# nelpy/ghost

Hardware: AMD Instinct MI355X
Metric: Msamples/s CWT (128ch x 1e6 samp x 100 scales); % HBM roofline; 1/2/4/8 GPU (higher is better)
Workload: dtype f32

## Files before the change

ghost_amd/csrc/api.cpp:

```cpp
#include <hip/hip_runtime.h>

#include <algorithm>
#include <cmath>
#include <cstdio>
#include <cstdlib>
#include <cstring>
#include <exception>
#include <map>
#include <new>
#include <string>
#include <vector>

#include "../../include/ghostcwt.h"
#include "../../include/ghostcwt_debug.h"
#include <memory>

#include "errors.h"
#include "host_out.h"
#include "interp.h"
#include "kernels.h"
#include "morse_exact.h"
#include "morlet_exact.h"
#include "options.h"
#include "planner.h"
// ... 1038 lines not shown
      }
      if (p->detect) {
        hipEvent_t bands_done;
        int rc_ = get_event(p, &bands_done);
        if (rc_) return rc_;
        he = hipEventRecord(bands_done, st);
        if (he == hipSuccess) he = hipStreamWaitEvent(p->det_stream, bands_done, 0);
        if (he != hipSuccess) return hip_err(he, "detector fork");
        he = launch_band_sums(p->d_hist, P1, p->d_bands, slots, p->det_stream);
        if (he != hipSuccess) return hip_err(he, "launch_band_sums");
        he = launch_precision_predict(p->d_bands, p->d_gain, p->d_scale_level, p->d_scale_length, p->ep_dev[ep.batch_first].pred_levels, S,
                                      (int)hp.levels.size(), (double)Pt, p->kappa_eps, p->oob_tol, p->d_pred, nullptr, nullptr, slots, psegs,
                                      p->det_stream);
        if (he != hipSuccess) return hip_err(he, "launch_precision_predict");
        p->last_batch_slots = slots; p->last_batch = ep.batch_first; p->last_pt = (double)Pt; p->last_rows = P1;
      }
    } else if (A > 1) {
      return set_err(GCWT_ERR_UNSUPPORTED, "internal: long mode without the float64 forward transform");
    } else {
    RUN(ST_FWD, launch_fft_cols_batch(dx, p->d_x, P1, kRowLen, N, P, P1 > 1 ? P : 0, p->d_tw4096,
                                      fast_fft ? p->d_tw256 : nullptr, p->d_sums, inv_n, sin, nb, st,
                                      rows_a));
    RUN(ST_FWD, launch_fft_rows(-1, p->d_x, p->d_x, kRowLen, rows_a, kRowLen, kRowLen, P, P, 0,
                                p->d_tw4096, fast_fft ? p->d_tw256 : nullptr, 1.0f, slots, st,
                                hp.n_fullband > 0 ? kRowLen : kRowLen / 2, hermitian ? P1 : 0));
    }
    const bool fused_blocks = p->fuse_blocks && p->synth_kernel == 7 && !p->use_synth16;
    const bool side = p->level_streams && hp.levels.size() > 2;
    const EpochDev& dev = p->ep_dev[ep.batch_first];
    std::vector<char> in_h(hp.levels.size(), 0);
    bool any_h = false;
    for (size_t l = 0; l < hp.levels.size(); ++l)
      if (level_kernel(p, hp.levels[l]) == LK_INTERP) {
        in_h[hp.levels[l].xr_owner >= 0 ? (size_t)hp.levels[l].xr_owner : l] = 1;
        any_h = true;
      }
    for (size_t l = 0; l < hp.levels.size(); ++l)
      if (hp.levels[l].xr_owner >= 0) in_h[l] = in_h[(size_t)hp.levels[l].xr_owner];
    const bool early = side && p->early_interp && p->profiling != 1 && !p->synth_streams && any_h &&
                       dev.n_items_i + dev.n_items_p[0] + dev.n_items_p[1] > 0;
    std::vector<int> stream_of(hp.levels.size(), 0);
    if (side) {
      double load[3] = {0.0, 0.0, 0.0};
      std::vector<size_t> order;
      for (size_t l = 0; l < hp.levels.size(); ++l)
        if (hp.levels[l].xr_owner == (int)l && !(early && in_h[l])) order.push_back(l);
      std::stable_sort(order.begin(), order.end(), [&](size_t a, size_t b) { return ep.lv[a].m > ep.lv[b].m; });
      const int k0 = early ? 1 : 0;
      for (size_t l : order) {
        const int k = (int)(std::min_element(load + k0, load + 3) - load);
        stream_of[l] = k;
        load[k] += 40e-6 + 32.0 * (double)ep.lv[l].m * (double)slots / 4.5e12;
      }
      for (size_t l = 0; l < hp.levels.size(); ++l) stream_of[l] = stream_of[hp.levels[l].xr_owner];
    }
    bool forked[2] = {false, false};
    hipEvent_t spectrum_ready = nullptr;
    if (side) {
      int rc_ = get_event(p, &spectrum_ready);
      if (rc_) return rc_;
      he = hipEventRecord(spectrum_ready, st);
      if (he != hipSuccess) return hip_err(he, "hipEventRecord");
    }
    for (size_t li = 0; li < (early ? 2 : 1) * hp.levels.size(); ++li) {
      const size_t l = li % hp.levels.size();
      if (early && (in_h[l] != 0) != (li < hp.levels.size())) continue;
      const LevelPlan& lp = hp.levels[l];
      const EpochLevel& el = ep.lv[l];
      float2* xr = p->d_xr + el.xr_offset;
      hipStream_t ls = st;
      RowTaper taper;
      if (p->high_precision && lp.taper_hi > 0.0 && lp.band_shift == 0) {
        const double k1 = lp.taper_hi * (double)Pt / (2.0 * M_PI), k0 = 0.5 * k1;
        if (k1 - k0 >= 1.0) { taper.p1 = P1; taper.k0 = (float)k0; taper.inv_width = (float)(1.0 / (k1 - k0)); }
      }
      if (side) {
        const int k = stream_of[l];
        ls = k == 0 ? st : p->aux[k - 1];
        if (k > 0 && !forked[k - 1]) {
          he = hipStreamWaitEvent(ls, spectrum_ready, 0);
          if (he != hipSuccess) return hip_err(he, "hipStreamWaitEvent");
          forked[k - 1] = true;
        }
        p->cur = ls;
      }
      if (lp.xr_owner != (int)l) {
      } else if (lp.decimation / A <= kMaxTwoPassDecimation) {
        const int Q = kRowLen * A / lp.decimation;
        const float2* src = p->d_x;
        int64_t src_row = kRowLen, src_cstride = P;
        if (lp.band_shift > 0) {
          const int64_t U = (int64_t)lp.band_shift * el.m / hp.block;
          if (U % P1 != 0 || U / P1 > Q) return set_err(GCWT_ERR_INVALID, "internal: band shift does not slice the spectrum");
          float2* xs = p->d_xs + (int64_t)stream_of[l] * slots * p->xs_stride;
          RUN(ST_DECIM, launch_shift_gather(p->d_x, xs, P1, Q, (int)(U / P1), kRowLen, P, p->xs_stride, slots, ls));
          src = xs; src_row = Q; src_cstride = p->xs_stride;
        }
        RUN(ST_DECIM, launch_fft_rows(+1, src, xr, Q, P1, src_row, Q, src_cstride, hp.max_xr,
                                      P1 > 1 ? el.m : 0, p->d_tw4096,
                                      fast_fft ? p->d_tw256 : nullptr, 1.0f, slots, ls, 0, 0, taper));
        if (P1 > 1)
          RUN(ST_DECIM, launch_fft_cols(+1, false, xr, xr, P1, Q, hp.max_xr, hp.max_xr, 0,
                                        p->d_tw4096, fast_fft ? p->d_tw256 : nullptr, p->d_sums,
                                        inv_n, 0, slots, ls));
      } else {
        const int n1 = (int)std::min<int64_t>(P1, el.m);
        const int q = (int)(el.m / n1);
        RUN(ST_DECIM, launch_level_small(p->d_x, xr, n1, q, kRowLen, P, hp.max_xr, p->d_tw4096, slots, ls, taper));
      }
      const float scale = (float)(1.0 / ((double)hp.block * (double)Pt));
      const LevelKernel lk = level_kernel(p, lp);
      if (lk == LK_SYNTH16 || (lk == LK_SYNTH7 && !fused_blocks))
        RUN(ST_BLOCK, launch_block_fft(xr, p->d_xb + el.xb_offset, el.m, lp.hop, lp.halo, el.blk_lo,
                                       el.nblk, hp.max_xr, hp.max_xb, p->d_tw256, scale, slots, ls));
    }
    if (side) p->cur = nullptr;
    auto join_levels = [&]() -> int {
      for (int k = 0; k < 2; ++k) {
        if (!forked[k]) continue;
        forked[k] = false;
        hipEvent_t done;
        int rc_ = get_event(p, &done);
        if (rc_) return rc_;
        he = hipEventRecord(done, p->aux[k]);
        if (he == hipSuccess) he = hipStreamWaitEvent(st, done, 0);
        if (he != hipSuccess) return hip_err(he, "level streams join");
      }
      return GCWT_OK;
    };
    if (!early) {
      int rc_ = join_levels();
      if (rc_) return rc_;
    }
    hipStream_t si = st;
    if (dev.n_items_i > 0) {
      const bool beside = p->synth_streams && (dev.n_items7 > 0 || dev.n_items7w > 0 || dev.n_items7n > 0 || dev.n_items > 0);
      if (beside) {
        hipEvent_t levels_done;
        int rc_ = get_event(p, &levels_done);
        if (rc_) return rc_;
        he = hipEventRecord(levels_done, st);
        if (he == hipSuccess) he = hipStreamWaitEvent(p->aux[0], levels_done, 0);
        if (he != hipSuccess) return hip_err(he, "synthesis fork");
        si = p->aux[0];
      }
      SynthiArgs ai{};
      ai.tw256 = p->d_tw256;
      ai.level_tw = p->d_level_tw;
      ai.items = dev.items_i;
      ai.levels = dev.levels_i;
      ai.scale_list = p->d_scale_list;
      ai.scale_aux = p->d_scale_aux;
      ai.gain = p->d_gain;
      ai.coef = p->d_interp_coef;
      ai.out = dout;
      ai.row_len = row_len;
      ai.xr = p->d_xr;
      ai.xr_cstride = hp.max_xr;
      ai.xb_scale = (float)(1.0 / ((double)hp.block * (double)Pt));
      ai.n_scales = S;
      ai.channels_fastest = p->interp_grid >= 0 ? p->interp_grid : (slots <= 32 ? 1 : 0);
      if (dev.n_items_i > 65535) ai.channels_fastest = 0;
      ai.seg = sout;
      p->cur = si;
      for (int part = 0; part < 2; ++part) {
        const int first = part == 0 ? 0 : dev.split_i, n_part = part == 0 ? dev.split_i : dev.n_items_i - dev.split_i;
        if (n_part == 0) continue;
        ai.items = dev.items_i + first;
        if (strided) RUN(ST_INTERP, launch_synthis(mode, ai, n_part, slots, si));
        else RUN(ST_INTERP, launch_synthi(mode, ai, n_part, slots, si));
      }
      p->cur = nullptr;
    }
    for (int k = 0; k < 2; ++k) {
      if (dev.n_items_p[k] == 0) continue;
      SynthpArgs ap{};
      ap.tw256 = p->d_tw256;
      ap.level_tw = p->d_level_tw;
      ap.items = dev.items_p[k];
      ap.levels = dev.levels_p;
      ap.scale_list = p->d_scale_list;
      ap.scale_aux = p->d_scale_aux;
      ap.gain_lv = p->d_gain_lv;
      ap.level_half_tw = p->d_half_tw;
      ap.coef = p->d_interp_coef;
      ap.out = dout;
      ap.row_len = row_len;
      ap.xr = p->d_xr;
      ap.xr_cstride = hp.max_xr;
      ap.xb_scale = (float)(1.0 / ((double)hp.block * (double)Pt));
      ap.n_scales = S;
      ap.channels_fastest = p->interp_grid >= 0 ? p->interp_grid : (slots <= 32 ? 1 : 0);
      if (dev.n_items_p[k] > 65535) ap.channels_fastest = 0;
      ap.flags = 0;
      ap.seg = sout;
      p->cur = si;
#ifdef GCWT_MEASURE
      if (strided) return set_err(GCWT_ERR_UNSUPPORTED, "output stride with the pipelined interpolating kernel");
      RUN(ST_INTERP, launch_synthp(mode, ap, dev.n_items_p[k], slots, k == 1, si));
#else
      return set_err(GCWT_ERR_INVALID, "internal: a level planned for the measure build's pipelined kernel");
#endif
      p->cur = nullptr;
    }
    if (early) {
      int rc_ = join_levels();
      if (rc_) return rc_;
    }
    if (dev.n_items > 0) {
      SynthArgs a{};
      a.xb = p->d_xb;
      a.bank = p->d_bank;
      a.tw256 = p->d_tw256;
      a.level_tw = p->d_level_tw;
      a.items = dev.items;
      a.levels = dev.levels;
      a.out = dout;
      a.xb_cstride = hp.max_xb;
      a.row_len = row_len;
      a.n_scales = S;
      a.seg = sout;
      RUN(ST_SYNTH, launch_synth(mode, a, dev.n_items, slots, st));
    }
    for (int variant = 0; variant < 3; ++variant) {
      const int wide = variant == 2;
      const int cols7 = variant == 0 ? 16 : p->synth_cols;
      const int n7 = variant == 0 ? dev.n_items7n : wide ? dev.n_items7w : dev.n_items7;
      if (n7 == 0) continue;
      Synth7Args a7{};
      a7.xb = p->d_xb;
      a7.bank = p->d_bank;
      a7.tw256 = p->d_tw256;
      a7.level_tw = p->d_level_tw;
      a7.items = variant == 0 ? dev.items7n : wide ? dev.items7w : dev.items7;
      a7.levels = dev.levels7;
      a7.scale_list = p->d_scale_list;
      a7.gain = p->d_gain;
      a7.gain_lv = p->d_gain_lv;
      a7.level_half_tw = p->d_half_tw;
      a7.complex_gains = hp.morlet ? 1 : 0;
      a7.out = dout;
      a7.xb_cstride = hp.max_xb;
      a7.row_len = row_len;
      a7.n_scales = S;
      a7.drop_stores = p->drop_stores;
      a7.seg = sout;
      a7.clock_probe = p->d_probe;
      if (fused_blocks) {
        a7.xr = p->d_xr;
        a7.xr_cstride = hp.max_xr;
        a7.xb_scale = (float)(1.0 / ((double)hp.block * (double)Pt));
      }
      if (strided) {
        RUN(ST_SYNTH, launch_synth7s(mode, cols7, a7, n7, slots, st));
        continue;
      }
#ifdef GCWT_MEASURE
      if (p->synth_kernel == 8 && variant == 1)
        RUN(ST_SYNTH, launch_synth8(mode, p->synth_cols, a7, n7, slots, st));
      else
#endif
        RUN(ST_SYNTH, launch_synth7(mode, cols7, wide != 0, a7, n7, slots, st));
    }
    if (si != st) {
      hipEvent_t interp_done;
      int rc_ = get_event(p, &interp_done);
      if (rc_) return rc_;
      he = hipEventRecord(interp_done, si);
      if (he == hipSuccess) he = hipStreamWaitEvent(st, interp_done, 0);
      if (he != hipSuccess) return hip_err(he, "synthesis join");
    }
    if (p->detect && p->d_y) {
      hipEvent_t pred_done;
      int rc_ = get_event(p, &pred_done);
      if (rc_) return rc_;
      he = hipEventRecord(pred_done, p->det_stream);
      if (he == hipSuccess) he = hipStreamWaitEvent(st, pred_done, 0);
      if (he != hipSuccess) return hip_err(he, "detector join");
    }
    if (p->profiling && !hp.levels.empty()) p->last.synth_launches++;
    auto response = [&](int i, int scratch, const float2** h_out) -> int {
      const auto cached = p->hfull_cache.find({i, P1});
      if (cached != p->hfull_cache.end()) { *h_out = cached->second; return GCWT_OK; }
      float2* dst = p->d_hfull + (int64_t)scratch * hp.max_p;
      float2* keep = nullptr;
      const int64_t bytes = (int64_t)sizeof(float2) * P;
      if (!p->hfull_cache_full && p->hfull_cache_bytes + bytes <= p->fullband_cache_cap) {
        if (hipMalloc((void**)&keep, (size_t)bytes) == hipSuccess) dst = keep;
        else {
          (void)hipGetLastError();
          p->hfull_cache_full = true;
        }
      }
      {
        SpanGuard sg_(p, ST_FULLBAND);
        int rc_ = sg_.rc;
        if (!rc_) {
          he = launch_fullband_filter(dst, p->d_bank_sc, i, p->d_amps, P1, st);
          if (he != hipSuccess) rc_ = hip_err(he, "launch_fullband_filter");
        }
        if (!rc_) rc_ = sg_.end();
        if (rc_) { if (keep) (void)hipFree(keep); return rc_; }
      }
      if (keep) {
        p->hfull_cache[{i, P1}] = keep;
        p->hfull_cache_bytes += bytes;
// ... 697 lines not shown
```

ghost_amd/csrc/kernels.h:

```cpp
#pragma once
#include <hip/hip_runtime.h>

#include <algorithm>
#include <cstdint>

#include "../../include/ghostcwt.h"

namespace gcwt {

constexpr int kRowLenDev = 4096;

#ifdef GCWT_MEASURE
constexpr bool kMeasureBuild = true;
#else
constexpr bool kMeasureBuild = false;
#endif

struct BankScale {
  double omega;
  double half_delay;
  int64_t length;
  int64_t amp_offset;
  int32_t bin_lo, n_bins;
  int32_t decimation;
// ... 17 lines not shown

inline int direct_front_pad(int64_t length) { return (int)((7 - (length - 1) / 2) & 7); }

constexpr int kSegBatch = 16;
struct SegIn {
  int64_t x_off[kSegBatch];
  int64_t n_valid[kSegBatch];
  int64_t n_lead[kSegBatch];
  int64_t ramp_lo[kSegBatch], ramp_hi[kSegBatch];
  int32_t n_channels, pad;
};
struct OutStride {
  int64_t r0 = 0;
  int64_t c0 = 0;
  int32_t k = 1;
  uint32_t magic = 0;
};
inline OutStride make_out_stride(int64_t k, int64_t r0) {
  OutStride o;
  o.r0 = r0;
  o.k = (int32_t)k;
  o.c0 = (r0 + k - 1) / k;
  o.magic = k > 1 ? (uint32_t)((((uint64_t)1 << 32) + (uint64_t)k - 1) / (uint64_t)k) : 0u;
  return o;
}
__device__ __forceinline__ bool stride_keep(const OutStride& o, int64_t n, int64_t* col) {
  const uint32_t t = (uint32_t)n;
  const uint32_t q = __umulhi(t, o.magic);
  *col = (int64_t)q - o.c0;
  return n >= 0 && q * (uint32_t)o.k == t;
}

struct SegOut {
  int64_t seg_col[kSegBatch];
  int64_t w_lo[kSegBatch];
  int64_t w_hi[kSegBatch];
  int32_t n_channels, pad;
  OutStride os;
};

struct SynthItemDev {
  int32_t level, scale, blk0, nblk;
};

struct SynthLevelDev {
  int32_t decimation, hop, halo, blk_base;
  int64_t xb_offset;
  int64_t tw_offset;
};

struct SynthArgs {
  const float2* xb;
  const float2* bank;
  const float2* tw256;
  const float2* level_tw;
  const SynthItemDev* items;
  const SynthLevelDev* levels;
  float* out;
  int64_t xb_cstride;
  int64_t row_len;
  int32_t n_scales;
  int32_t pad;
  SegOut seg;
};

struct Synth7Item {
  int32_t level, blk0, rtile, pad;
};

struct Synth7Level {
  int32_t decimation, log2r, hop, halo, nblk, n_scales, scale_offset, blk_base;
  int32_t n_plain;
  int32_t half_offset;
  int32_t band_shift;
  int32_t pad1;
  int64_t xb_offset;
  int64_t tw_offset;
  int64_t xr_offset;
  int64_t m_mask;
};

struct Synth7Args {
  const float2* xb;
  const float2* bank;
  const float2* tw256;
  const float2* level_tw;
  const Synth7Item* items;
  const Synth7Level* levels;
  const int32_t* scale_list;
  const float* gain;
  const float* gain_lv;
  const float2* level_half_tw;
  float* out;
  int64_t xb_cstride;
  int64_t row_len;
  const float2* xr;
  int64_t xr_cstride;
  float xb_scale;
  int32_t complex_gains;
  unsigned long long* clock_probe;
  int32_t n_scales;
  int32_t drop_stores;
  SegOut seg;
};

__host__ __device__ constexpr int synth7_ex_elem(int lg, int colw, int j) {
  return ((colw >> lg) << (4 + lg)) + (colw & ((1 << lg) - 1)) + (j << lg);
}
__host__ __device__ constexpr bool synth7_exchange_wave_local(int ncol, int R) { return R <= ncol && 16 * R <= 64; }
constexpr bool synth7_exchange_spans_one_wave(int ncol, int lg) {
  for (int colw = 0; colw < ncol; ++colw)
    for (int j = 0; j < 16; ++j)
      if ((16 * colw) >> 6 != synth7_ex_elem(lg, colw, j) >> 6) return false;
  return true;
}
constexpr int kSynth7LocalStride = 4;
#define GCWT_EX_CHECK(ncol, lg, local)                                                                    \
  static_assert(synth7_exchange_wave_local(ncol, 1 << (lg)) == (local) &&                                 \
                    ((1 << (lg)) > (ncol) || synth7_exchange_spans_one_wave(ncol, lg) == (local)) &&      \
                    (((1 << (lg)) > (ncol) ? (ncol) : (1 << (lg))) <= kSynth7LocalStride) == (local),     \
                "k_synth7: the wave-local predicate does not match the column mapping")
GCWT_EX_CHECK(16, 0, true);  GCWT_EX_CHECK(16, 1, true);  GCWT_EX_CHECK(16, 2, true);  GCWT_EX_CHECK(16, 3, false);
GCWT_EX_CHECK(16, 4, false); GCWT_EX_CHECK(16, 5, false); GCWT_EX_CHECK(16, 6, false);
GCWT_EX_CHECK(32, 0, true);  GCWT_EX_CHECK(32, 1, true);  GCWT_EX_CHECK(32, 2, true);  GCWT_EX_CHECK(32, 3, false);
GCWT_EX_CHECK(32, 4, false); GCWT_EX_CHECK(32, 5, false); GCWT_EX_CHECK(32, 6, false); GCWT_EX_CHECK(32, 7, false);
#undef GCWT_EX_CHECK

hipError_t launch_synth7(int mode, int ncol, bool wide_halo, const Synth7Args& a, int n_items, int n_channels,
                         hipStream_t st);
hipError_t launch_synth7s(int mode, int ncol, const Synth7Args& a, int n_items, int n_channels, hipStream_t st);

struct SynthiItem {
  int32_t level, blk0;
  int32_t pass0, n_pass;
  int32_t wt_lo, wt_hi;
};
struct SynthiLevel {
  int32_t decimation, q, log2q, factor;
  int32_t hop, halo, nblk, n_scales, scale_offset, blk_base;
  int32_t log2nb, taps;
  int64_t tw_offset;
  int64_t xr_offset;
  int64_t m_mask;
  int64_t coef_offset;
};
struct SynthiArgs {
  const float2* tw256;
  const float2* level_tw;
  const SynthiItem* items;
  const SynthiLevel* levels;
  const int32_t* scale_list;
  const int32_t* scale_aux;
  const float* gain;
  const float* coef;
  float* out;
  int64_t row_len;
  const float2* xr;
  int64_t xr_cstride;
  float xb_scale;
  int32_t n_scales;
  int32_t channels_fastest;
  SegOut seg;
};
hipError_t launch_synthi(int mode, const SynthiArgs& a, int n_items, int n_channels, hipStream_t st);
hipError_t launch_synthis(int mode, const SynthiArgs& a, int n_items, int n_channels, hipStream_t st);
constexpr int kSynthpThreads = 512;
constexpr int kSynthpProducers = 2;
constexpr int kSynthpSlots = 4;
constexpr int kSynthpMaxFactor = 256;
struct SynthpItem {
  int32_t level, blk0;
  int32_t round0, n_rounds;
};
struct SynthpLevel {
  int32_t decimation, factor;
  int32_t hop, halo, nblk, n_scales, scale_offset, blk_base;
  int32_t log2nb;
  int32_t n_plain;
  int32_t half_offset;
  int32_t help;
  int64_t tw_offset;
  int64_t xr_offset;
  int64_t m_mask;
  int64_t coef_offset;
};
struct SynthpArgs {
  const float2* tw256;
  const float2* level_tw;
  const SynthpItem* items;
  const SynthpLevel* levels;
  const int32_t* scale_list;
  const int32_t* scale_aux;
  const float* gain_lv;
  const float2* level_half_tw;
  const float* coef;
  float* out;
  int64_t row_len;
  const float2* xr;
  int64_t xr_cstride;
  float xb_scale;
  int32_t n_scales;
  int32_t channels_fastest;
  int32_t flags;
  int32_t pad0;
  SegOut seg;
};
hipError_t launch_synthp(int mode, const SynthpArgs& a, int n_items, int n_channels, bool exact0, hipStream_t st);
hipError_t launch_synth8(int mode, int ncol, const Synth7Args& a, int n_items, int n_channels,
                         hipStream_t st);

hipError_t dft_f64(const double* x, int64_t n, int is_complex, int inverse, double* out);
hipError_t fastconv_f64(const double* signal, int64_t n, int signal_is_complex, const double* kernel, int64_t m,
                        int kernel_is_complex, int64_t first, int64_t count, double* out);

hipError_t rows_to_host(const float* d_src, int64_t src_pitch, int64_t n_rows, int64_t row_elems, void* dst,
                        int64_t dst_pitch, bool widen, bool pinned);

constexpr int kSumParts = 256;
constexpr int kSumPartsOwn = 64;
constexpr size_t channel_sum_doubles(size_t n_channels) { return n_channels * (kSumParts + 1); }
hipError_t launch_channel_sum(const float* x, int64_t n, int n_channels, double* sums,
                              hipStream_t st);
hipError_t launch_build_bank(float2* bank, float* gain, const BankScale* sc, const double* amps,
                             int n_scales, int B, hipStream_t st);
constexpr int kScaleIndexMask = 0x00FFFFFF;
hipError_t launch_scale_windows(const float* gain, int32_t* scale_list, int n_listed, float tol,
                                float* gain_lv, bool prune, hipStream_t st);
hipError_t launch_gain_rows_complex(const float2* bank, const int32_t* scale_list, int n_listed, float2* gain_lv,
                                    hipStream_t st);
hipError_t launch_bank_gain(const float2* bank, float* gain, const BankScale* sc, int n_scales,
                            hipStream_t st);
hipError_t launch_fullband_filter(float2* h, const BankScale* sc, int scale, const double* amps,
                                  int p1, hipStream_t st);
hipError_t launch_fullband_mul(const float2* x, const float2* h, float2* z, int64_t p, int n_slots,
                               hipStream_t st);
constexpr int kFullbandSet = 4;
struct FullbandSet {
  const float2* h[kFullbandSet];
  float2* z[kFullbandSet];
  int32_t n, pad;
};
hipError_t launch_fullband_rows(const float2* x, const FullbandSet& set, int p1, int64_t x_cstride, int64_t z_cstride,
                                const float2* twt, const float2* tw256, int n_slots, hipStream_t st,
                                int group = 0);
bool fullband_cols_fused(int p1);
constexpr int kFullband4Scales = 8;
hipError_t launch_fullband4(int mode, const float2* x, const float2* const* h, const int32_t* scales, int n, float* out,
                            int64_t x_cstride, const float2* twt, const float2* tw256, int n_scales, int64_t row_len,
                            const SegOut& seg, int n_slots, hipStream_t st);
hipError_t launch_fullband_cols(int mode, const float2* z, float* out, int p1, int64_t z_cstride,
                                const float2* tw4096, const float2* tw256, int scale, int n_scales,
                                int64_t row_len, const SegOut& seg, int n_slots, hipStream_t st);
hipError_t launch_fullband_store(int mode, const float2* y, float* out, int64_t p, int scale,
                                 int n_scales, int64_t row_len, const SegOut& seg, int n_segments,
                                 hipStream_t st);
hipError_t launch_build_direct(float2* psi, const DirectScale* sc, int n_direct, int64_t max_len,
                               const double* amps, float2* tail, float2* psi_literal, hipStream_t st);
hipError_t launch_fft_cols(int sign, bool real_in, const void* in, float2* out, int len, int ld,
                           int64_t in_cstride, int64_t out_cstride, int64_t tw_n,
                           const float2* tw4096, const float2* tw256, const double* sums, double inv_n, int64_t n_valid,
                           int n_channels, hipStream_t st, int64_t n_lead = 0, int rows_out = 0);
hipError_t launch_fft_cols_batch(const float* in, float2* out, int len, int ld, int64_t in_cstride,
                                 int64_t out_cstride, int64_t tw_n, const float2* tw4096,
                                 const float2* tw256, const double* sums, double inv_n,
                                 const SegIn& segs, int n_segments, hipStream_t st, int rows_out);
struct RowTaper {
  int32_t p1 = 0;
  float k0 = 0.f, inv_width = 0.f;
};
hipError_t launch_fft_rows(int sign, const float2* in, float2* out, int len, int64_t n_rows,
                           int64_t in_ld, int64_t out_ld, int64_t in_cstride, int64_t out_cstride,
                           int64_t tw_n, const float2* tw4096, const float2* tw256, float scale,
                           int n_channels, hipStream_t st, int out_len = 0, int mirror = 0,
                           RowTaper taper = RowTaper());
void fwd64_fill_tables(double2* host);
hipError_t launch_fwd64_cols(const float* in, double2* y, int p1, int64_t in_cstride, int64_t y_cstride,
                             int64_t p, const double2* tables, const double* sums, double inv_n,
                             const SegIn& segs, int n_segments, int rows_out, hipStream_t st, int in_stride = 1,
                             int in_offset = 0, bool fold_mean = false);
hipError_t launch_channel_sum_final(double* sums, int n_channels, int parts, hipStream_t st);
constexpr int fold_parts(int p1) { return p1 == 256 ? 32 : 256; }
hipError_t launch_fwd64_rows(const double2* y, float2* x, int n_rows, int64_t y_cstride, int64_t x_cstride,
                             const double2* tables, int n_slots, int out_len, int mirror, hipStream_t st,
                             int comb_a = 0, int comb_n = 1, int64_t p_true = 0, float* hist = nullptr, int hist_rows = 0,
                             const double* fold_sums = nullptr, double inv_n = 0.0, int64_t n_valid = 0, int p1 = 0);

constexpr int kSpecBands = 16 * 24;
__host__ __device__ inline int spec_band(float k) {
  union { float f; uint32_t u; } b;
  b.f = k;
  const int v = (int)(b.u >> 19) - 127 * 16;
  return v < 0 ? 0 : (v >= kSpecBands ? kSpecBands - 1 : v);
}
struct PredSegs {
  int32_t seg[kSegBatch];
  int32_t n_channels, pad;
};
struct PredLevel {
  int32_t decimation;
  int32_t band_shift;
  float k0, k1;
};
constexpr int kRowBands = 128;
hipError_t launch_band_sums(const float* hist, int p1, float* bands, int n_slots, hipStream_t st);
hipError_t launch_precision_predict(const float* bands, const float* gain, const int32_t* scale_level,
                                    const int32_t* scale_length, const PredLevel* levels, int n_scales, int n_levels, double p_true,
// ... 50 lines not shown
```

ghost_amd/csrc/synthi.hip:

```cpp
#include <hip/hip_runtime.h>

#include <type_traits>

#include "interp.h"
#include "kernels.h"
#include "options.h"
#include "synth_math.h"

#ifndef GCWT_STORE_AUX
#define GCWT_STORE_AUX 2
#endif

namespace gcwt {

namespace {
constexpr int kT = kInterpTaps;
static_assert(kT == 8, "the FIR loop below is written for 8 taps");
constexpr int kColsI = kInterpCols;
constexpr int kLgColsI = kColsI == 32 ? 5 : kColsI == 16 ? 4 : 3;
constexpr int kThreadsI = 16 * kColsI;
constexpr int kWavesI = kThreadsI / 64;
constexpr int kPlaneI = kThreadsI + 1;
constexpr int kZPad = 4;
constexpr int kSlotsMax = kColsI / 2;
static_assert(kColsI == kInterpCols, "the host cuts the passes for this many columns (interp.h)");
constexpr int kZElems = 256 * kColsI + kSlotsMax * kZPad;
constexpr int kExElems = kZElems > 16 * kPlaneI ? kZElems : 16 * kPlaneI;
constexpr int kGainRowI = 16 * 20;
constexpr int kLdsBytes = kExElems * 8 + 256 * 8 + kSlotsMax * kGainRowI * 4 + 2 * 256 * 4;

__device__ __forceinline__ v2f fir_mul_re(v2f z, v2f c) {
  v2f r;
  asm("v_pk_mul_f32 %0, %1, %2 op_sel:[0,0] op_sel_hi:[0,1]" : "=v"(r) : "v"(z), "v"(c));
  return r;
}
__device__ __forceinline__ v2f fir_mul_im(v2f z, v2f c) {
  v2f r;
  asm("v_pk_mul_f32 %0, %1, %2 op_sel:[1,0] op_sel_hi:[1,1]" : "=v"(r) : "v"(z), "v"(c));
  return r;
}
__device__ __forceinline__ v2f fir_fma_re(v2f acc, v2f z, v2f c) {
  v2f r;
  asm("v_pk_fma_f32 %0, %1, %2, %3 op_sel:[0,0,0] op_sel_hi:[0,1,1]" : "=v"(r) : "v"(z), "v"(c), "v"(acc));
  return r;
}
__device__ __forceinline__ v2f fir_fma_im(v2f acc, v2f z, v2f c) {
  v2f r;
  asm("v_pk_fma_f32 %0, %1, %2, %3 op_sel:[1,0,0] op_sel_hi:[1,1,1]" : "=v"(r) : "v"(z), "v"(c), "v"(acc));
  return r;
}
__device__ __forceinline__ v2f pk_mul(v2f a, v2f b) {
  v2f r;
  asm("v_pk_mul_f32 %0, %1, %2" : "=v"(r) : "v"(a), "v"(b));
  return r;
}
__device__ __forceinline__ v2f pk_fma(v2f a, v2f b, v2f c) {
  v2f r;
  asm("v_pk_fma_f32 %0, %1, %2, %3" : "=v"(r) : "v"(a), "v"(b), "v"(c));
  return r;
}
template <int J0, int J1>
__device__ __forceinline__ void fir_taps(const v2f* zp, const v2f (&cf)[2][kT], v2f (&are)[2], v2f (&aim)[2]) {
  {
    const v2f w = zp[J0];
#pragma unroll
    for (int pr = 0; pr < 2; ++pr) { are[pr] = fir_mul_re(w, cf[pr][J0]); aim[pr] = fir_mul_im(w, cf[pr][J0]); }
  }
#pragma unroll
  for (int j = J0 + 1; j < J1; ++j) {
    const v2f w = zp[j];
#pragma unroll
    for (int pr = 0; pr < 2; ++pr) { are[pr] = fir_fma_re(are[pr], w, cf[pr][j]); aim[pr] = fir_fma_im(aim[pr], w, cf[pr][j]); }
  }
}
}

template <int MODE>
__global__ void __launch_bounds__(kThreadsI, kColsI == 32 ? 4 : 3) k_synthi(const SynthiArgs a) {
  extern __shared__ __attribute__((aligned(16))) char smem[];
  v2f* const ex = reinterpret_cast<v2f*>(smem);
  v2f* const twl = ex + kExElems;
  float* const stage = reinterpret_cast<float*>(twl + 256);
  int* const sc_lds = reinterpret_cast<int*>(stage + kSlotsMax * kGainRowI);
  int* const aux_lds = sc_lds + 256;

  const SynthiItem it = a.items[a.channels_fastest ? blockIdx.y : blockIdx.x];
  const SynthiLevel lv = a.levels[it.level];
  const int c = a.channels_fastest ? blockIdx.x : blockIdx.y;
  const int seg = c / a.seg.n_channels, ch = c - seg * a.seg.n_channels;
  const int R = lv.decimation, q = lv.q, lgq = lv.log2q, hop = lv.hop, halo = lv.halo;
  const int lgnb = lv.log2nb, nb = 1 << lgnb;
  const int64_t n_b = (int64_t)(lv.blk_base + it.blk0) * hop * R;
  const int64_t w_lo = a.seg.w_lo[seg];
  const int64_t w_len = a.seg.w_hi[seg] - w_lo;
  if (n_b + (int64_t)nb * hop * R <= w_lo || n_b >= w_lo + w_len) return;

  const int tid = threadIdx.x, lane = tid & 63;
  const int wave = __builtin_amdgcn_readfirstlane(tid >> 6);
  const int colw = tid >> 4, t = tid & 15;
  const int lgns = kLgColsI - lgq - lgnb, ns = 1 << lgns;
  const int zslot = colw >> lgq, p = colw & (q - 1);
  const int slot = zslot & (ns - 1), blk_l = zslot >> lgns;
  const int nzs = kColsI >> lgq;
  const int n_scales = lv.n_scales;
  const int* const scales = a.scale_list + lv.scale_offset;
  const int* const auxs = a.scale_aux + lv.scale_offset;
  for (int i = tid; i < n_scales; i += kThreadsI) { sc_lds[i] = scales[i]; aux_lds[i] = auxs[i]; }
  if (tid < 256) {
    const float2 w = a.tw256[tid];
    twl[tid] = (v2f){w.x, w.y};
  }
  auto stage_slot = [&](int i) { return (i >> 8) * kGainRowI + (i & 15) * 20 + ((i >> 4) & 15); };
  for (int i = tid; i < ns * 256; i += kThreadsI) {
    const int sb = min(it.pass0 * ns + (i >> 8), n_scales - 1);
    stage[stage_slot(i)] = a.gain[(int64_t)(scales[sb] & kScaleIndexMask) * 256 + (i & 255)];
  }

  v2f* const fx = ex;
  v2f* const xbs = ex + kSlotsMax * 256;
  {
    v2f v[16];
    if (colw < nb) {
      const int64_t base = (int64_t)(lv.blk_base + min(it.blk0 + colw, lv.nblk - 1)) * hop - halo + t;
      const float2* xr = a.xr + (int64_t)c * a.xr_cstride + lv.xr_offset;
#pragma unroll
      for (int j = 0; j < 16; ++j) {
        const float2 u = xr[(base + 16 * j) & lv.m_mask];
        v[j] = (v2f){u.x, -u.y};
      }
      idft16v(v);
#pragma unroll
      for (int m = 0; m < 16; ++m) {
        const float2 w = a.tw256[(t * m) & 255];
        fx[colw * 256 + t * 16 + (m ^ t)] = cmulv(v[dft16_pos(m)], (v2f){w.x, w.y});
      }
    }
    __syncthreads();
    if (colw < nb) {
#pragma unroll
      for (int k1 = 0; k1 < 16; ++k1) v[k1] = fx[colw * 256 + k1 * 16 + (t ^ k1)];
      idft16v(v);
#pragma unroll
      for (int j = 0; j < 16; ++j) {
        const v2f z = v[dft16_pos(j)];
        xbs[colw * 256 + t + 16 * j] = (v2f){z.x * a.xb_scale, -z.y * a.xb_scale};
      }
    }
    __syncthreads();
  }
  v2f pw[16];
  {
    const int r = p * lv.factor;
    const float2* ltw = a.level_tw + lv.tw_offset;
    const float2 b0 = ltw[t * r], st = ltw[16 * r];
    v2f wcur = (v2f){b0.x, b0.y};
    const v2f wstep = (v2f){st.x, st.y};
#pragma unroll
    for (int j = 0; j < 16; ++j) {
      pw[j] = cmulv(xbs[blk_l * 256 + t + 16 * j], wcur);
      wcur = cmulv(wcur, wstep);
    }
  }

  const int a2 = tid >> kLgColsI, col2 = tid & (kColsI - 1);
  const int zslot2 = col2 >> lgq, p2 = col2 & (q - 1);
  const int zstride = (256 << lgq) + kZPad;
  v2f* const zw = ex + zslot2 * zstride + (a2 << lgq) + p2;

  const int I = lv.factor;
  const bool six = lv.taps == 6;
  int lgi4 = 0;
  while ((4 << lgi4) < I) ++lgi4;
  const int tps = hop * (R >> 2);
  const int n_wt = it.wt_hi - it.wt_lo;
  static_assert(GCWT_SYNTHI_COLS != 16 || (kWavesI == 4 && kInterpMaxFactor <= 1024),
                "a wave's lane-tasks keep their class mod I / 4 (the 8- and 32-column measurement builds: I <= 256 only)");
  const float* const coef_lv = a.coef + lv.coef_offset;
  constexpr int kElem = 1;
  const unsigned ext_bytes = w_len > 0 ? (unsigned)(w_len * (4 * kElem)) : 0u;
  float* const out0 = a.out + ((int64_t)ch * a.n_scales * a.row_len + a.seg.seg_col[seg] + w_lo) * kElem;
  const int s_base = (int)(n_b - w_lo);
  const int pass_end = it.pass0 + it.n_pass;
  int cur_par = -1;
  v2f cf[2][kT];
  __syncthreads();

  for (int pass = it.pass0; pass < pass_end; ++pass) {
    const int b0 = pass * ns;
    const bool has_next = pass + 1 < pass_end;
    float nxt[kSlotsMax];
    if (has_next) {
#pragma unroll
      for (int u = 0; u < kSlotsMax; ++u) {
        const int i = tid + kThreadsI * u;
        if (i < ns * 256) {
          const int sb = min(b0 + ns + (i >> 8), n_scales - 1);
          nxt[u] = a.gain[(int64_t)(sc_lds[sb] & kScaleIndexMask) * 256 + (i & 255)];
        }
      }
    }
    {
      const int bs = min(b0 + slot, n_scales - 1);
      const int entry = sc_lds[bs];
      const int kc = aux_lds[bs] & 0xffff;
      const float4* const hs = reinterpret_cast<const float4*>(stage + slot * kGainRowI + t * 20);
      v2f v[16];
      unsigned cut = (unsigned)__builtin_amdgcn_readfirstlane(entry) >> 24;
      if (q == 2) {
        const int other = sc_lds[min(b0 + (((colw ^ 2) >> lgq) & (ns - 1)), n_scales - 1)];
        cut = min(cut, (unsigned)__builtin_amdgcn_readfirstlane(min((unsigned)entry >> 24, (unsigned)other >> 24)));
        cut = (unsigned)__builtin_amdgcn_readfirstlane(cut);
      }
      switch (cut) {
#define GCWT_WINDOW(hi) case 16 - (hi): gain_first_layer<hi>(v, pw, hs); break;
        GCWT_WINDOW(15) GCWT_WINDOW(14) GCWT_WINDOW(13) GCWT_WINDOW(12) GCWT_WINDOW(11) GCWT_WINDOW(10) GCWT_WINDOW(9)
#undef GCWT_WINDOW
        default: gain_first_layer<16>(v, pw, hs); break;
      }
      idft16v_tail(v);
      const unsigned step8 = (unsigned)((t - kc) & 255) << 3;
      unsigned idx8 = (unsigned)((-(kc >> lgq) * p) & 255) << 3;
      v2f* const exw = ex + ((t - kc) & 15) * kPlaneI + colw;
      const char* const twb = reinterpret_cast<const char*>(twl);
#pragma unroll
      for (int j = 0; j < 16; ++j) {
        exw[j * kColsI] = cmulv(v[dft16_pos(j)], *reinterpret_cast<const v2f*>(twb + idx8));
        idx8 = (idx8 + step8) & 0x7f8u;
      }
    }
    __syncthreads();
    if (has_next) {
#pragma unroll
      for (int u = 0; u < kSlotsMax; ++u) {
        const int i = tid + kThreadsI * u;
        if (i < ns * 256) stage[stage_slot(i)] = nxt[u];
      }
    }
    {
      v2f v[16];
#pragma unroll
      for (int k1 = 0; k1 < 16; ++k1) v[k1] = ex[k1 * kPlaneI + tid];
      __syncthreads();
      idft16v(v);
#pragma unroll
      for (int m1 = 0; m1 < 16; ++m1) zw[(16 * m1) << lgq] = v[dft16_pos(m1)];
    }
    __syncthreads();

    {
      for (int zi = 0; zi < nzs; ++zi) {
        const int sl = zi & (ns - 1), bl = zi >> lgns;
        if (b0 + sl >= n_scales || it.blk0 + bl >= lv.nblk) continue;
        const int entry = __builtin_amdgcn_readfirstlane(sc_lds[b0 + sl]);
        const int par = (__builtin_amdgcn_readfirstlane(aux_lds[b0 + sl]) >> 16) & 1;
        const int wt0 = (wave - zi * n_wt) & (kWavesI - 1);
        const int key = par | (lgi4 > 6 ? (wt0 & ((1 << (lgi4 - 6)) - 1)) << 1 : 0);
        if (key != cur_par) {
          const int sigma = (wt0 * 64 + lane) & ((1 << lgi4) - 1);
          const float4* const cp = reinterpret_cast<const float4*>(coef_lv + ((int64_t)par * I + sigma * 4) * kT);
#pragma unroll
          for (int pr = 0; pr < 2; ++pr) {
            const float4 a0 = cp[4 * pr], a1 = cp[4 * pr + 1], b0 = cp[4 * pr + 2], b1 = cp[4 * pr + 3];
            cf[pr][0] = (v2f){a0.x, b0.x}; cf[pr][1] = (v2f){a0.y, b0.y}; cf[pr][2] = (v2f){a0.z, b0.z}; cf[pr][3] = (v2f){a0.w, b0.w};
            cf[pr][4] = (v2f){a1.x, b1.x}; cf[pr][5] = (v2f){a1.y, b1.y}; cf[pr][6] = (v2f){a1.z, b1.z}; cf[pr][7] = (v2f){a1.w, b1.w};
          }
          cur_par = key;
        }
        const int srow = entry & kScaleIndexMask;
        const uint64_t dst_bits = reinterpret_cast<uint64_t>(out0 + (int64_t)srow * a.row_len * kElem);
        const uint32_t dst_lo = __builtin_amdgcn_readfirstlane((uint32_t)dst_bits);
        const uint32_t dst_hi = __builtin_amdgcn_readfirstlane((uint32_t)(dst_bits >> 32));
        float* const dst = reinterpret_cast<float*>(((uint64_t)dst_hi << 32) | dst_lo);
        const __amdgpu_buffer_rsrc_t rsrc = __builtin_amdgcn_make_buffer_rsrc(
            dst, 0, __builtin_amdgcn_readfirstlane(ext_bytes), 0x00020000);
        const v2f* const zs = ex + zi * zstride + (halo << lgq) - (kT / 2 - 1);
        const int s_blk = s_base + bl * hop * R;
        const int wt_a = max(it.wt_lo, s_blk >= 0 ? 0 : (-s_blk) >> 8);
        const int wt_b = (int)min((int64_t)it.wt_hi, max((int64_t)0, (w_len - s_blk + 255) >> 8));
        const int f_lo = max(wt_a, s_blk >= 0 ? 0 : (255 - s_blk) >> 8);
        const int f_hi = (int)min((int64_t)min(wt_b, tps >> 6), max((int64_t)0, (w_len - s_blk) >> 8));
        auto edge_task = [&](int wt) {
          const int k = wt * 64 + lane;
          if (k < tps) {
            const v2f* const zp = zs + (k >> lgi4);
            v2f are[2], aim[2];
            if (six) fir_taps<1, kT - 1>(zp, cf, are, aim);
            else fir_taps<0, kT>(zp, cf, are, aim);
            float res[4];
#pragma unroll
            for (int pr = 0; pr < 2; ++pr) {
              const v2f p2v = pk_fma(aim[pr], aim[pr], pk_mul(are[pr], are[pr]));
              res[2 * pr] = MODE == GCWT_OUT_AMPLITUDE_F32 ? __builtin_amdgcn_sqrtf(p2v.x) : p2v.x;
              res[2 * pr + 1] = MODE == GCWT_OUT_AMPLITUDE_F32 ? __builtin_amdgcn_sqrtf(p2v.y) : p2v.y;
            }
            const int s0 = s_blk + 4 * k;
#pragma unroll
            for (int i = 0; i < 4; ++i)
              if ((unsigned)(s0 + i) < (unsigned)w_len)
                __builtin_amdgcn_raw_buffer_store_b32(__builtin_bit_cast(unsigned, res[i]), rsrc,
                                                      (unsigned)(s0 + i) * 4u, 0, GCWT_STORE_AUX);
          }
        };
        int wt = wt_a + ((wt0 - wt_a) & (kWavesI - 1));
        for (; wt < min(f_lo, wt_b); wt += kWavesI) edge_task(wt);
        if (wt < f_hi) {
          const v2f* zp = zs + ((wt * 64 + lane) >> lgi4);
          const int z_step = (64 * kWavesI) >> lgi4;
          unsigned soff = (unsigned)(s_blk + 256 * wt) * 4u;
          const unsigned voff = (unsigned)lane * 16u;
          typedef unsigned v4u __attribute__((ext_vector_type(4)));
          auto whole_task = [&](auto taps) {
            v2f are[2], aim[2];
            if constexpr (decltype(taps)::value == 6) fir_taps<1, kT - 1>(zp, cf, are, aim);
            else fir_taps<0, kT>(zp, cf, are, aim);
            v4u pk;
#pragma unroll
            for (int pr = 0; pr < 2; ++pr) {
              const v2f p2v = pk_fma(aim[pr], aim[pr], pk_mul(are[pr], are[pr]));
              pk[2 * pr] = __builtin_bit_cast(unsigned, MODE == GCWT_OUT_AMPLITUDE_F32 ? __builtin_amdgcn_sqrtf(p2v.x) : p2v.x);
              pk[2 * pr + 1] = __builtin_bit_cast(unsigned, MODE == GCWT_OUT_AMPLITUDE_F32 ? __builtin_amdgcn_sqrtf(p2v.y) : p2v.y);
            }
            __builtin_amdgcn_raw_buffer_store_b128(pk, rsrc, voff, soff, GCWT_STORE_AUX);
            zp += z_step;
            soff += 1024u * kWavesI;
          };
          if (six) for (; wt < f_hi; wt += kWavesI) whole_task(std::integral_constant<int, 6>());
          else for (; wt < f_hi; wt += kWavesI) whole_task(std::integral_constant<int, 8>());
        }
        for (; wt < wt_b; wt += kWavesI) edge_task(wt);
      }
    }
    __syncthreads();
  }
}

hipError_t launch_synthi(int mode, const SynthiArgs& a, int n_items, int n_channels, hipStream_t st) {
  if (n_items == 0) return hipSuccess;
  if (mode != GCWT_OUT_AMPLITUDE_F32 && mode != GCWT_OUT_POWER_F32) return hipErrorInvalidValue;
  static bool attr_done[64] = {};
  int dev_ = 0;
  (void)hipGetDevice(&dev_);
  bool& attr_set = attr_done[dev_ & 63];
  if (!attr_set) {
    hipError_t e = hipFuncSetAttribute((const void*)k_synthi<GCWT_OUT_AMPLITUDE_F32>,
                                       hipFuncAttributeMaxDynamicSharedMemorySize, kLdsBytes);
    if (e != hipSuccess) return e;
    e = hipFuncSetAttribute((const void*)k_synthi<GCWT_OUT_POWER_F32>,
                            hipFuncAttributeMaxDynamicSharedMemorySize, kLdsBytes);
    if (e != hipSuccess) return e;
    attr_set = true;
  }
  if ((a.channels_fastest ? n_items : n_channels) > 65535) return hipErrorInvalidValue;
  const dim3 grid = a.channels_fastest ? dim3(n_channels, n_items) : dim3(n_items, n_channels), block(kThreadsI);
  int lds = kLdsBytes;
  if (kMeasureBuild && option_is_set("synthi_pad_kb")) {
    lds += 1024 * (int)option_or("synthi_pad_kb", 0);
    hipError_t e = hipFuncSetAttribute((const void*)k_synthi<GCWT_OUT_AMPLITUDE_F32>, hipFuncAttributeMaxDynamicSharedMemorySize, lds);
    if (e == hipSuccess) e = hipFuncSetAttribute((const void*)k_synthi<GCWT_OUT_POWER_F32>, hipFuncAttributeMaxDynamicSharedMemorySize, lds);
    if (e != hipSuccess) return e;
  }
  if (mode == GCWT_OUT_AMPLITUDE_F32)
    hipLaunchKernelGGL((k_synthi<GCWT_OUT_AMPLITUDE_F32>), grid, block, lds, st, a);
  else
    hipLaunchKernelGGL((k_synthi<GCWT_OUT_POWER_F32>), grid, block, lds, st, a);
  return hipGetLastError();
}

}
```

Baseline: 9817.

## Vectorize gain staging with per-level gain table and hoist prologue loads

Gain rows are now read as float4 vectors from a per-level pre-gathered table (gain_lv), replacing scalar gathers through the scale index. Table, twiddle and level-twiddle loads are issued early into registers and written to LDS after the input loads, so their latency overlaps. The first-stage twiddle multiply now reads the LDS twiddle table instead of global memory. When the halo is wide enough, the two edge rows of the inverse DFT output are not stored. This relies on host code populating d_gain_lv (not shown) and adds register pressure.

Result: no change. 9806 (-0.1%).

```diff
diff --git a/ghost_amd/csrc/api.cpp b/ghost_amd/csrc/api.cpp
--- a/ghost_amd/csrc/api.cpp
+++ b/ghost_amd/csrc/api.cpp
@@ -1214,6 +1214,7 @@
       ai.scale_list = p->d_scale_list;
       ai.scale_aux = p->d_scale_aux;
       ai.gain = p->d_gain;
+      ai.gain_lv = p->d_gain_lv;
       ai.coef = p->d_interp_coef;
       ai.out = dout;
       ai.row_len = row_len;
diff --git a/ghost_amd/csrc/kernels.h b/ghost_amd/csrc/kernels.h
--- a/ghost_amd/csrc/kernels.h
+++ b/ghost_amd/csrc/kernels.h
@@ -193,6 +193,7 @@
   const int32_t* scale_list;
   const int32_t* scale_aux;
   const float* gain;
+  const float* gain_lv;
   const float* coef;
   float* out;
   int64_t row_len;
diff --git a/ghost_amd/csrc/synthi.hip b/ghost_amd/csrc/synthi.hip
--- a/ghost_amd/csrc/synthi.hip
+++ b/ghost_amd/csrc/synthi.hip
@@ -105,16 +105,39 @@
   const int n_scales = lv.n_scales;
   const int* const scales = a.scale_list + lv.scale_offset;
   const int* const auxs = a.scale_aux + lv.scale_offset;
-  for (int i = tid; i < n_scales; i += kThreadsI) { sc_lds[i] = scales[i]; aux_lds[i] = auxs[i]; }
-  if (tid < 256) {
-    const float2 w = a.tw256[tid];
-    twl[tid] = (v2f){w.x, w.y};
-  }
-  auto stage_slot = [&](int i) { return (i >> 8) * kGainRowI + (i & 15) * 20 + ((i >> 4) & 15); };
-  for (int i = tid; i < ns * 256; i += kThreadsI) {
-    const int sb = min(it.pass0 * ns + (i >> 8), n_scales - 1);
-    stage[stage_slot(i)] = a.gain[(int64_t)(scales[sb] & kScaleIndexMask) * 256 + (i & 255)];
-  }
+  constexpr int kTab = (256 + kThreadsI - 1) / kThreadsI;
+  int sc_v[kTab], aux_v[kTab];
+  float2 tw_v[kTab];
+#pragma unroll
+  for (int u = 0; u < kTab; ++u) {
+    const int i = tid + kThreadsI * u;
+    sc_v[u] = i < n_scales ? scales[i] : 0;
+    aux_v[u] = i < n_scales ? auxs[i] : 0;
+    tw_v[u] = i < 256 ? a.tw256[i] : make_float2(0.f, 0.f);
+  }
+  constexpr int kRowVec = 64;
+  static_assert(kSlotsMax * kRowVec <= 2 * kThreadsI, "at most two 16-byte loads per thread and pass");
+  const float4* const gain_rows = reinterpret_cast<const float4*>(a.gain_lv) + (int64_t)lv.scale_offset * kRowVec;
+  const int n_gvec = ns * kRowVec;
+  float4 g_v0 = make_float4(0.f, 0.f, 0.f, 0.f), g_v1 = g_v0;
+  auto load_one = [&](int pass, int f) {
+    return gain_rows[min(pass * ns + (f >> 6), n_scales - 1) * kRowVec + (f & 63)];
+  };
+  auto load_gains = [&](int pass) {
+    if (tid < n_gvec) g_v0 = load_one(pass, tid);
+    if (kThreadsI + tid < n_gvec) g_v1 = load_one(pass, kThreadsI + tid);
+  };
+  auto park_one = [&](int f, const float4& g) {
+    *reinterpret_cast<float4*>(stage + (f >> 6) * kGainRowI + ((f >> 2) & 15) * 20 + (f & 3) * 4) = g;
+  };
+  auto park_gains = [&]() {
+    if (tid < n_gvec) park_one(tid, g_v0);
+    if (kThreadsI + tid < n_gvec) park_one(kThreadsI + tid, g_v1);
+  };
+  load_gains(it.pass0);
+  const int p_r = p * lv.factor;
+  const float2* const ltw = a.level_tw + lv.tw_offset;
+  const float2 ltw_b0 = ltw[t * p_r], ltw_st = ltw[16 * p_r];
 
   v2f* const fx = ex;
   v2f* const xbs = ex + kSlotsMax * 256;
@@ -128,17 +151,23 @@
         const float2 u = xr[(base + 16 * j) & lv.m_mask];
         v[j] = (v2f){u.x, -u.y};
       }
+    }
+#pragma unroll
+    for (int u = 0; u < kTab; ++u) {
+      const int i = tid + kThreadsI * u;
+      if (i < n_scales) { sc_lds[i] = sc_v[u]; aux_lds[i] = aux_v[u]; }
+      if (i < 256) twl[i] = (v2f){tw_v[u].x, tw_v[u].y};
+    }
+    park_gains();
+    if (colw < nb) {
       idft16v(v);
 #pragma unroll
-      for (int m = 0; m < 16; ++m) {
-        const float2 w = a.tw256[(t * m) & 255];
-        fx[colw * 256 + t * 16 + (m ^ t)] = cmulv(v[dft16_pos(m)], (v2f){w.x, w.y});
-      }
+      for (int m = 0; m < 16; ++m) fx[colw * 256 + t * 16 + (m ^ t)] = v[dft16_pos(m)];
     }
     __syncthreads();
     if (colw < nb) {
 #pragma unroll
-      for (int k1 = 0; k1 < 16; ++k1) v[k1] = fx[colw * 256 + k1 * 16 + (t ^ k1)];
+      for (int k1 = 0; k1 < 16; ++k1) v[k1] = cmulv(fx[colw * 256 + k1 * 16 + (t ^ k1)], twl[(t * k1) & 255]);
       idft16v(v);
 #pragma unroll
       for (int j = 0; j < 16; ++j) {
@@ -150,11 +179,8 @@
   }
   v2f pw[16];
   {
-    const int r = p * lv.factor;
-    const float2* ltw = a.level_tw + lv.tw_offset;
-    const float2 b0 = ltw[t * r], st = ltw[16 * r];
-    v2f wcur = (v2f){b0.x, b0.y};
-    const v2f wstep = (v2f){st.x, st.y};
+    v2f wcur = (v2f){ltw_b0.x, ltw_b0.y};
+    const v2f wstep = (v2f){ltw_st.x, ltw_st.y};
 #pragma unroll
     for (int j = 0; j < 16; ++j) {
       pw[j] = cmulv(xbs[blk_l * 256 + t + 16 * j], wcur);
@@ -166,6 +192,7 @@
   const int zslot2 = col2 >> lgq, p2 = col2 & (q - 1);
   const int zstride = (256 << lgq) + kZPad;
   v2f* const zw = ex + zslot2 * zstride + (a2 << lgq) + p2;
+  const bool z_trim = halo - (kT / 2 - 1) >= 16 && 256 - halo + kT / 2 < 240;
 
   const int I = lv.factor;
   const bool six = lv.taps == 6;
@@ -188,17 +215,7 @@
   for (int pass = it.pass0; pass < pass_end; ++pass) {
     const int b0 = pass * ns;
     const bool has_next = pass + 1 < pass_end;
-    float nxt[kSlotsMax];
-    if (has_next) {
-#pragma unroll
-      for (int u = 0; u < kSlotsMax; ++u) {
-        const int i = tid + kThreadsI * u;
-        if (i < ns * 256) {
-          const int sb = min(b0 + ns + (i >> 8), n_scales - 1);
-          nxt[u] = a.gain[(int64_t)(sc_lds[sb] & kScaleIndexMask) * 256 + (i & 255)];
-        }
-      }
-    }
+    if (has_next) load_gains(pass + 1);
     {
       const int bs = min(b0 + slot, n_scales - 1);
       const int entry = sc_lds[bs];
@@ -229,21 +246,21 @@
       }
     }
     __syncthreads();
-    if (has_next) {
-#pragma unroll
-      for (int u = 0; u < kSlotsMax; ++u) {
-        const int i = tid + kThreadsI * u;
-        if (i < ns * 256) stage[stage_slot(i)] = nxt[u];
-      }
-    }
+    if (has_next) park_gains();
     {
       v2f v[16];
 #pragma unroll
       for (int k1 = 0; k1 < 16; ++k1) v[k1] = ex[k1 * kPlaneI + tid];
       __syncthreads();
-      idft16v(v);
-#pragma unroll
-      for (int m1 = 0; m1 < 16; ++m1) zw[(16 * m1) << lgq] = v[dft16_pos(m1)];
+      if (z_trim) {
+        idft16v(v);
+#pragma unroll
+        for (int m1 = 1; m1 < 15; ++m1) zw[(16 * m1) << lgq] = v[dft16_pos(m1)];
+      } else {
+        idft16v(v);
+#pragma unroll
+        for (int m1 = 0; m1 < 16; ++m1) zw[(16 * m1) << lgq] = v[dft16_pos(m1)];
+      }
     }
     __syncthreads();
 
```
